# sushruta/uniformgrid-raytracing

Hardware: AMD Instinct MI355X
Metric: Mrays/s (primary+shadow+1-bounce) (higher is better)
Workload: dtype f32

## Files before the change

### uniformgrid-raytracing_amd/csrc/ugrt_context.hip

```cpp
#include "ugrt_ctx.h"

static int check_device(int device)
{
	int n = 0;
	hipError_t e = hipGetDeviceCount(&n);
	if (e != hipSuccess || n <= 0)
		return ugrt_fail(UGRT_ENODEV, "no HIP device available (%s); libugrt has no CPU fallback",
				 e != hipSuccess ? hipGetErrorString(e) : "device count 0");
	if (device < 0 || device >= n)
		return ugrt_fail(UGRT_EINVAL, "device %d out of range (%d devices)", device, n);
	return UGRT_OK;
}

int ugrt_buf_reserve(ugrt_ctx *ctx, DevBuf &b, size_t bytes)
{
	if (bytes <= b.cap && b.p)
		return UGRT_OK;
	size_t want = bytes + bytes / 2;
	if (want < 256)
		want = 256;
	void *np = nullptr;
	hipError_t e = hipMalloc(&np, want);
	if (e != hipSuccess)
		return ugrt_fail(UGRT_ENOMEM, "hipMalloc(%zu) failed: %s", want, hipGetErrorString(e));
// ... 145 lines not shown
	buf_free(ctx->pseg);
	buf_free(ctx->pbkt);
	buf_free(ctx->sray);
	if (ctx->h_pinned)
		(void)hipHostFree(ctx->h_pinned);
	if (ctx->d_small)
		(void)hipFree(ctx->d_small);
	for (int s = 0; s < UGRT_ST_COUNT; s++)
		for (auto &p : ctx->prof[s]) {
			(void)hipEventDestroy(p.a);
			(void)hipEventDestroy(p.b);
		}
	for (auto &p : ctx->prof_pool) {
		(void)hipEventDestroy(p.a);
		(void)hipEventDestroy(p.b);
	}
	delete ctx;
}

static const struct {
	const char *key;
	int lo, hi;
} k_opt[UGRT_OPT_COUNT] = {
	{ "dda_rays_per_wave", 0, 64 }, { "dda_coop", 1, 1 << 30 },     { "dda_kernel", 0, 1 },
	{ "dda_cull_min", 1, 1 << 30 }, { "dda_blocks", 1, 1 << 20 },
	{ "primary_seg", 64, 1 << 20 }, { "shadow_beam", 64, 8192 },
	{ "shadow_xseg", 64, 1 << 20 }, { "shadow_sizebits", 0, 8 },    { "shadow_itemsort", 0, 1 },
	{ "shadow_mbits", 1, 24 },      { "shadow_key64", 0, 1 },       { "sort_library", 0, 1 },
	{ "async_build", 0, 1 },        { "primary_waves", 64, 1 << 20 },
	{ "shadow_waves", 64, 1 << 20 }, { "dda_sort", 0, 1 }, { "primary_order", 0, 1 }, { "primary_chunk", 4, 64 }, { "sort_items", 8, 16 }, { "dda_cull_work", 1, 1 << 30 },
	{ "dda_split", 0, 4 }, { "dda_split_load", 50, 100000 }, { "dda_split_segments", 1, 4 }, { "primary_xcd_run", 0, 4096 }, { "shadow_xcd_run", 0, 4096 },
	{ "primary_centre", 0, 1 }, { "sort_rank", 0, 1 }, { "ray_sort", 0, 1 }, { "shadow_sieve", 0, 64 },
	{ "any_rays_per_wave", 0, 64 }, { "any_coop", 1, 1 << 30 }, { "uniform_reuse", 0, 1 },
	{ "light_reuse", 0, 1 }, { "shadow_pairs", 0, 1 },
};

extern "C" int ugrt_ctx_get_state(ugrt_ctx *ctx, const char *key, long long *value)
{
	if (!ctx || !key || !value)
		return ugrt_fail(UGRT_EINVAL, "ctx_get_state: null argument");
	if (strcmp(key, "radix_launches") == 0)
		*value = (long long)ctx->rs_launches;
	else if (strcmp(key, "sort_rank_atomic") == 0)
		*value = ctx->rs_atomic_rank < 0 ? -1 : (ctx->rs_atomic_rank == 1 && ctx->opt[UGRT_OPT_SORT_RANK] != 0 ? 1 : 0);
	else if (strcmp(key, "shadow_key_bits") == 0)
		*value = (long long)ctx->shadow_key_bits;
	else if (strcmp(key, "shadow_pairs_counted") == 0)
		*value = ctx->shadow_pairs_counted ? 1 : 0;
	else if (strcmp(key, "primary_deferred_merges") == 0)
		*value = (long long)ctx->merges_deferred;
	else if (strcmp(key, "primary_completed_merges") == 0)
		*value = (long long)ctx->merges_completed;
	else if (strcmp(key, "primary_merge_pending") == 0)
		*value = ctx->grid[UGRT_GRID_PERSPECTIVE].valid && ctx->grid[UGRT_GRID_PERSPECTIVE].merge_pending ? 1 : 0;
	else if (strcmp(key, "uniform_builds_reused") == 0)
		*value = (long long)ctx->uniform_reused;
	else if (strcmp(key, "light_builds_reused") == 0)
		*value = (long long)ctx->light_reused;
	else if (strcmp(key, "primary_slots_unarmed") == 0) {
		const size_t ncell = (size_t)ctx->nbx * (size_t)ctx->nby;
		std::vector<u64> b((size_t)ctx->npix);
		std::vector<u32> d(ncell);
		UGRT_HIP(hipSetDevice(ctx->device));
		UGRT_HIP(hipStreamSynchronize(ctx->stream));
		UGRT_HIP(hipMemcpy(b.data(), ctx->best.p, b.size() * sizeof(u64), hipMemcpyDeviceToHost));
		UGRT_HIP(hipMemcpy(d.data(), ctx->pdone.p, d.size() * sizeof(u32), hipMemcpyDeviceToHost));
		long long bad = 0;
		for (u64 v : b)
			bad += v != ~0ull;
		for (u32 v : d)
			bad += v != 0u;
		*value = bad;
	} else if (strcmp(key, "recip_mismatches") == 0) {
		unsigned long long bad = 0;
		const int rc = ugrt_recip_selftest(ctx, &bad);
		if (rc != UGRT_OK)
			return rc;
		*value = (long long)bad;
	} else if (strcmp(key, "f2i_mismatches") == 0) {
		unsigned long long bad = 0;
		const int rc = ugrt_f2i_selftest(ctx, &bad);
// ... 21 lines not shown
				return ugrt_fail(UGRT_EINVAL, "ctx_set_option: %s %d outside [%d,%d]", key, value, k_opt[i].lo,
						 k_opt[i].hi);
			ctx->opt[i] = (value < 0 || ((i == UGRT_OPT_DDA_RPW || i == UGRT_OPT_ANY_RPW) && value == 0)) ? -1 : value;
			return UGRT_OK;
		}
	return ugrt_fail(UGRT_EINVAL, "ctx_set_option: unknown key '%s'", key);
}

extern "C" int ugrt_ctx_set_stream(ugrt_ctx *ctx, void *hip_stream)
{
	if (!ctx)
		return ugrt_fail(UGRT_EINVAL, "set_stream: null ctx");
	UGRT_HIP(hipStreamSynchronize(ctx->stream));
	ctx->stream = (hipStream_t)hip_stream;
	return UGRT_OK;
}

extern "C" int ugrt_ctx_synchronize(ugrt_ctx *ctx)
{
	if (!ctx)
		return ugrt_fail(UGRT_EINVAL, "synchronize: null ctx");
	UGRT_HIP(hipStreamSynchronize(ctx->stream));
	if (ugrt_reported_status(ctx) != 0u || ctx->overflow_seen) {
		const unsigned bits = ugrt_reported_status(ctx);
		ctx->overflow_seen = false;
		for (int g = 0; g < 3; g++)
			ctx->h_pinned[UGRT_PIN_REPORT + 4 * g + 3] = 0u;
		ctx->h_pinned[UGRT_PIN_SHADOW + 2] = 0u;
		UGRT_HIP(hipMemsetAsync(ctx->d_small + UGRT_DSMALL_STATUS, 0, 4, ctx->stream));
		UGRT_HIP(hipStreamSynchronize(ctx->stream));
		for (int g = 0; g < 3; g++)
			ctx->grid[g].have_est = false;
		ctx->have_shadow_est = false;
		ctx->overflow_repair = true;
		return ugrt_fail(UGRT_EOVERFLOW, "an asynchronous call needed more room than its estimate gave it (status %u: "
						  "1 grid build, 2 shadow candidate pairs, 4 shadow work items): the frames since the last "
						  "synchronisation are incomplete, repeat them", bits);
	}
	ctx->overflow_repair = false;
	return UGRT_OK;
}

struct TexArg {
	float v[100];
};
__global__ void k_store_table(TexArg t, float *dst)
{
	int i = threadIdx.x;
	if (i < 100)
		dst[i] = t.v[i];
}

float *ugrt_ctx_tex(ugrt_ctx *ctx)
{
	float *dst = (float *)(ctx->d_small + UGRT_DSMALL_TEX);
	if (ctx->tex_dirty) {
		TexArg t;
		memcpy(t.v, ctx->tex_host, sizeof(t.v));
		hipLaunchKernelGGL(k_store_table, dim3(1), dim3(128), 0, ctx->stream, t, dst);
		ctx->tex_dirty = false;
	}
	return dst;
}

extern "C" int ugrt_upload_camera(ugrt_ctx *ctx, const float camcoords[64])
{
	if (!ctx || !camcoords)
		return ugrt_fail(UGRT_EINVAL, "upload_camera: null argument");
	memcpy(ctx->cam.cc, camcoords, sizeof(float) * 64);
// ... 149 lines not shown
```

### uniformgrid-raytracing_amd/csrc/ugrt_ctx.h

```cpp
#ifndef UGRT_CTX_H
#define UGRT_CTX_H

#include <hip/hip_runtime.h>

#include <vector>

#include "ugrt_internal.h"

struct CamBlock {
	float cc[64];
	float light[4];
	int W, H, nbx, nby;
	int strict_tex;
};

enum {
	UGRT_OPT_DDA_RPW = 0,
	UGRT_OPT_DDA_COOP,
	UGRT_OPT_DDA_KERNEL,
	UGRT_OPT_DDA_CULL_MIN,
	UGRT_OPT_DDA_BLOCKS,
	UGRT_OPT_PRIMARY_SEG,
	UGRT_OPT_SHADOW_BEAM,
	UGRT_OPT_SHADOW_XSEG,
	UGRT_OPT_SHADOW_SIZEBITS,
	UGRT_OPT_SHADOW_ITEMSORT,
	UGRT_OPT_SHADOW_MBITS,
	UGRT_OPT_SHADOW_KEY64,
	UGRT_OPT_SORT_LIBRARY,
	UGRT_OPT_ASYNC_BUILD,
	UGRT_OPT_PRIMARY_WAVES,
	UGRT_OPT_SHADOW_WAVES,
	UGRT_OPT_DDA_SORT,
	UGRT_OPT_PRIMARY_ORDER,
	UGRT_OPT_PRIMARY_CHUNK,
	UGRT_OPT_SORT_ITEMS,
	UGRT_OPT_DDA_CULL_WORK,
	UGRT_OPT_DDA_SPLIT,
	UGRT_OPT_DDA_SPLIT_LOAD,
	UGRT_OPT_DDA_SPLIT_SEGMENTS,
	UGRT_OPT_PRIMARY_XCD_RUN,
	UGRT_OPT_SHADOW_XCD_RUN,
	UGRT_OPT_PRIMARY_CENTRE,
	UGRT_OPT_SORT_RANK,
	UGRT_OPT_RAY_SORT,
	UGRT_OPT_SHADOW_SIEVE,
	UGRT_OPT_ANY_RPW,
	UGRT_OPT_ANY_COOP,
	UGRT_OPT_UNIFORM_REUSE,
	UGRT_OPT_LIGHT_REUSE,
	UGRT_OPT_SHADOW_PAIRS,
	UGRT_OPT_COUNT
};

struct DevBuf {
	void *p = nullptr;
	size_t cap = 0;
};

struct Grid;
struct BuildPlan {
	Grid *G;
	int F, ny, nz, ylo, yhi;
	u32 C;
	unsigned long long active;
	u32 Rn, W, R;
	u32 *rw;
	u32 *report, *status;
	bool no_wide;
	bool own_sort;
	bool prehist;
};

struct Grid {
	DevBuf rng, sizes, scan;
	DevBuf parts;
	DevBuf wide;
	DevBuf key[2], val[2];
	DevBuf span, offset;
	DevBuf projz;
	DevBuf uspan;
	int slabs = 1, F = 0;
	u32 est_rn = 0, est_w = 0;
	bool have_est = false, async_pending = false, r_exact = true;
	bool waited = false;
	unsigned long long active_cells = 0;
	u32 *keys = nullptr, *vals = nullptr;
	u32 R = 0, C = 0, cells_used = 0;
	int dims[3] = { 0, 0, 0 };
	float ug[12] = { 0 };
	bool valid = false;
	const u32 *wide_zeroed = nullptr;
	bool merge_pending = false;
	BuildPlan merge_plan = {};
};

#define UGRT_DSMALL_DDA_RAYS 2
#define UGRT_DSMALL_DDA_RAYS_B 4
#define UGRT_DSMALL_TICKET 8
#define UGRT_DSMALL_STATUS 14
#define UGRT_DSMALL_SHADOW_WORK 16
#define UGRT_DSMALL_PAIRS 20
#define UGRT_DSMALL_TEX 32
#define UGRT_DSMALL_DDA 132
#define UGRT_DSMALL_RW 236
#define UGRT_DSMALL_SHADOW 254
#define UGRT_DSMALL_PRIMARY 264
#define UGRT_DSMALL_WORDS (132 + 104 + 28 + 32)
#define UGRT_PIN_RW 0
#define UGRT_PIN_CELLS_USED 4
#define UGRT_PIN_REFS 8
#define UGRT_PIN_PAIRS 10
#define UGRT_PIN_CHUNKS 11
#define UGRT_PIN_BEAMS 12
#define UGRT_PIN_SHADOW_WORK (UGRT_PIN_SHADOW + 4)
#define UGRT_PIN_REPORT 32
#define UGRT_PIN_SHADOW 44
#define UGRT_PIN_WORDS 64
#define UGRT_STATUS_BUILD_OVERFLOW 1u
#define UGRT_STATUS_PAIR_OVERFLOW 2u
#define UGRT_STATUS_ITEM_OVERFLOW 4u
#define UGRT_DDA_STATS 46
#define UGRT_PRIMARY_STATS 16
static_assert(UGRT_DSMALL_DDA + 2 * UGRT_DDA_STATS <= UGRT_DSMALL_RW, "the DDA's counters run into the build counts");
static_assert(UGRT_DSMALL_RW + 6 <= UGRT_DSMALL_SHADOW && UGRT_DSMALL_SHADOW + 10 <= UGRT_DSMALL_PRIMARY && UGRT_DSMALL_PRIMARY + 2 * UGRT_PRIMARY_STATS <= UGRT_DSMALL_WORDS && UGRT_PIN_SHADOW + 8 <= UGRT_PIN_WORDS && UGRT_PIN_REPORT + 12 <= UGRT_PIN_SHADOW, "scratch layout");

struct ProfPair {
	hipEvent_t a, b;
};

struct ugrt_ctx {
	ugrt_config cfg;
	int device = 0;
	hipStream_t stream = nullptr;
	CamBlock cam;
	float tex_host[100];
	bool tex_dirty = false;
	int nbx = 0, nby = 0;
	int face_lo = 0, face_hi = -1;
	int p0 = 0, npix = 0;
	Grid grid[3];
	DevBuf temp;
	DevBuf scan_state;
	u32 scan_epoch = 0;
	DevBuf rs_state, rs_tmp[2][2];
	u32 rs_tiles = 0;
	u32 rs_epoch = 0;
	bool batch_open = false;
	int nbatch = 0;
	BuildPlan batch[2];
	unsigned long long rs_launches = 0;
	bool rs_prehist = false;
	int rs_atomic_rank = -1;
	DevBuf trirec;
	const float *rec_verts = nullptr;
	const int *rec_tris = nullptr;
	int rec_faces = 0;
	bool rec_valid = false;
// ... 13 lines not shown
	const u32 *ubitmap_span = nullptr;
	DevBuf witems, wscan;
	DevBuf ubitmap;
	DevBuf dsort;
	DevBuf dsplit;
	u32 dda_turn = 0;
	u32 dsplit_rpw = 0, dsplit_turn = 0;
	bool dda_deeper_level = false;
	DevBuf best;
	DevBuf pdone;
	DevBuf rmap[2];
	DevBuf rstart, cbase;
	DevBuf skey[2], sval[2], sdesc, sstart, sbase;
	DevBuf tkey[2], tval[2], tbcnt;
	DevBuf sray;
	DevBuf citem;
	DevBuf pseg;
	DevBuf pbkt;
	bool shadow_pairs_counted = false;
	DevBuf sitem;
	u32 *h_pinned = nullptr;
	u32 *d_small = nullptr;
	unsigned prof_mask = 0;
	unsigned chunk_capacity = 0;
	const unsigned *chunk_prefix = nullptr, *chunk_map = nullptr;
	bool ray_sort_pending = false;
	int opt[UGRT_OPT_COUNT];
	std::vector<ProfPair> prof[UGRT_ST_COUNT];
	std::vector<ProfPair> prof_pool;
	bool overflow_seen = false;
	bool overflow_repair = false;
	u32 est_pairs = 0, est_beams = 0;
	bool have_shadow_est = false, shadow_async_pending = false;
	u32 shadow_key_bits = 0;
	unsigned long long stats[8] = { 0 };
	unsigned long long dda_stats[UGRT_DDA_STATS] = { 0 };
	unsigned long long primary_stats[UGRT_PRIMARY_STATS] = { 0 };
	unsigned long long merges_deferred = 0, merges_completed = 0;
};

#define UGRT_HIP(call)                                                                            \
	do {                                                                                      \
		hipError_t e_ = (call);                                                           \
		if (e_ != hipSuccess)                                                             \
			return ugrt_fail(UGRT_EHIP, "%s:%d %s -> %s", __FILE__, __LINE__, #call, \
					 hipGetErrorString(e_));                                  \
	} while (0)

int ugrt_buf_reserve(ugrt_ctx *ctx, DevBuf &b, size_t bytes);
static inline const float4 *ugrt_trirec_of(const ugrt_ctx *ctx, const float *d_vertlist, const int *d_trilist)
{
	const bool use_rec = ctx->rec_valid && ctx->rec_verts == d_vertlist && ctx->rec_tris == d_trilist;
	return use_rec ? (const float4 *)ctx->trirec.p : (const float4 *)nullptr;
}
int ugrt_slab_union(ugrt_ctx *ctx, const u32 *d_span, const u32 *d_offset, u32 C, u32 slabs, const u32 **uspan,
		    const u32 **uoffset);
int ugrt_grid_complete(ugrt_ctx *ctx, Grid &G);
float *ugrt_ctx_tex(ugrt_ctx *ctx);
static inline u32 ugrt_reported_status(const ugrt_ctx *ctx)
{
	const u32 *p = ctx->h_pinned;
	return p[UGRT_PIN_REPORT + 3] | p[UGRT_PIN_REPORT + 7] | p[UGRT_PIN_REPORT + 11] | p[UGRT_PIN_SHADOW + 2];
}
void ugrt_prof_begin(ugrt_ctx *ctx, int stage);
void ugrt_prof_end(ugrt_ctx *ctx, int stage);

// ... 36 lines not shown
```

### uniformgrid-raytracing_amd/csrc/ugrt_trace_shadow.hip

```cpp
#include <algorithm>
#include <cstdlib>
#include "ugrt_packet.h"
#include "ugrt_rs_hist.h"
#include "ugrt_scan.h"
#ifndef GCHUNK
#define GCHUNK 32u
#endif

struct GBox {
	float cx, cy, cz;
	float rx, ry, rz;
	u32 ray_start;
	u32 ray_count;
};

__device__ __forceinline__ u32 d_spread10(u32 v)
{
	v &= 0x3FFu;
	v = (v | (v << 16)) & 0x030000FFu;
	v = (v | (v << 8)) & 0x0300F00Fu;
	v = (v | (v << 4)) & 0x030C30C3u;
	v = (v | (v << 2)) & 0x09249249u;
	return v;
}
// ... 81 lines not shown
		float tVal = t_value_list[pixel];
		float rd[3];
		rd[0] = (cmPt[0] + tVal * ray_direction_list[pixel * 3 + 0]) - cam.cc[0];
		rd[1] = (cmPt[1] + tVal * ray_direction_list[pixel * 3 + 1]) - cam.cc[1];
		rd[2] = (cmPt[2] + tVal * ray_direction_list[pixel * 3 + 2]) - cam.cc[2];
		D_NORMALIZE(rd);
		code = KEY64 ? d_dir_morton(rd) : d_dir_oct(rd, (mbits + 1u) / 2u, mbits / 2u);
	}
	if (KEY64)
		((u64 *)keys)[i] = ((u64)cell << 30) | (u64)code;
	else
		((u32 *)keys)[i] = key32 = (cell << mbits) | code;
	vals[i] = pixel;
	}
	if (!KEY64 && hs.hist)
		d_rs_count(s_rsh, key32 & 0xFFu, i < n);
	}
	__syncthreads();
	d_rs_flush(s_rsh, hs);
}

template <typename K>
__global__ __launch_bounds__(WL_THREADS) void k_shadow_runs(const K *__restrict__ keys, u32 n, u32 shift,
							     u32 *__restrict__ rstart, u32 *__restrict__ rend)
{
	u32 i = blockIdx.x * WL_THREADS + threadIdx.x;
	if (i >= n)
		return;
	u32 c = (u32)(keys[i] >> shift);
	if (i == 0 || (u32)(keys[i - 1] >> shift) != c)
		rstart[c] = i;
	if (i == n - 1 || (u32)(keys[i + 1] >> shift) != c)
		rend[c] = i + 1;
}

struct ShadowCountLoad {
	const u32 *span, *rstart, *rend;
	u32 beam;
	unsigned long long *tests;
	bool ITEMS;
	__device__ __forceinline__ void operator()(u32 base, u32 C, u32 (&v)[SC_ITEMS]) const
	{
#pragma unroll
		for (int k = 0; k < SC_ITEMS; k++) {
			const u32 c = base + (u32)k;
			u32 x = 0;
			if (c < C) {
				const u32 g = (rend[c] - rstart[c] + beam - 1u) / beam, sp = span[c];
				x = ITEMS ? (sp + 63u) / 64u * ((g + GCHUNK - 1) / GCHUNK) : g;
				if (!ITEMS && g && sp)
					atomicAdd(tests, (unsigned long long)sp * (unsigned long long)g);
			}
			v[k] = x;
		}
	}
};

__device__ __forceinline__ u32 d_find_cell(const u32 *__restrict__ incl, u32 C, u32 x)
{
	u32 lo = 0, hi = C - 1;
	while (lo < hi) {
		u32 mid = (lo + hi) >> 1;
		if (incl[mid] > x)
			hi = mid;
		else
			lo = mid + 1;
// ... 668 lines not shown
		if (ok) {
			const u32 pos = end - old + rank;
			if (pos < out_cap)
				pair_tri[pos] = tri;
		}
	}
}

#ifdef UGRT_SHADOW_TIMELINE
__device__ unsigned long long *g_shadow_tl;
#endif
template <bool REC>
__global__ __launch_bounds__(64) void k_trace_shadow(CamBlock cam, const u32 *__restrict__ xincl, u32 G,
						      const u32 *__restrict__ item_seg, const u32 *__restrict__ item_sub,
						      const GBox *__restrict__ boxes, const u32 *__restrict__ pstart,
						      const u32 *__restrict__ pend, const u32 *__restrict__ pair_tri,
						      const float *__restrict__ verts, const int *__restrict__ tris,
						      const float4 *__restrict__ rec, const float *__restrict__ t_value_list,
						      const float *__restrict__ ray_direction_list,
						      int *__restrict__ is_shadowed, const u32 *__restrict__ ray_pixels,
						      const float *__restrict__ cmPt, u32 XSEG, u32 *__restrict__ sub_done,
						      u32 nsubmax, const float4 *__restrict__ sray, u32 item_cap,
						      u32 *__restrict__ report, const u32 *__restrict__ status,
						      const unsigned long long *__restrict__ work, u32 SLICES, u32 W0, u32 SIEVE, u32 NSIEVE)
{
	__shared__ __attribute__((aligned(16))) float lds[64 * 16];
	const int lane = threadIdx.x;
#ifdef UGRT_SHADOW_TIMELINE
	const unsigned long long tl0 = __builtin_amdgcn_s_memrealtime();
	u32 tl_n = 0;
#endif
	if (blockIdx.x == 0 && lane == 0) {
		report[2] = *status;
		report[3] = 0u;
		reinterpret_cast<unsigned long long *>(report + 4)[0] = work[0];
		reinterpret_cast<unsigned long long *>(report + 4)[1] = work[1];
	}
	const u32 total = item_cap;
	const float lx = cam.cc[0], ly = cam.cc[1], lz = cam.cc[2];
	u32 first = blockIdx.x;
	if (SLICES == 1u) {
		first = d_xcd_block();
	} else if (SLICES > 1u) {
		const u32 rl = (SLICES >> 1) - 1u, j = blockIdx.x >> 3;
		first = ((((j >> rl) << 3) + (blockIdx.x & 7u)) << rl) + (j & ((1u << rl) - 1u));
	}
	const bool persistent = SLICES == 1u;
	for (u32 base = first; base < (persistent ? total : W0 + NSIEVE); base += gridDim.x) {
		const bool sieve = !persistent && base >= W0;
		const u32 n_v = sieve ? SIEVE : 1u, stride_v = sieve ? NSIEVE : 0u;
		u32 sgm_v = XSEG_LAST + 1u, gs_v = 0u;
		const u32 my_it = base + (u32)lane * stride_v;
		if ((u32)lane < n_v && my_it < total) {
			sgm_v = item_seg[my_it];
			gs_v = item_sub[my_it];
		}
		const u32 flagged_v = __hip_atomic_load(sub_done + (size_t)(gs_v >> 7) * nsubmax + (gs_v & 127u), __ATOMIC_RELAXED, __HIP_MEMORY_SCOPE_AGENT);
		unsigned long long todo = __ballot(sgm_v <= XSEG_LAST && flagged_v == 0u);
	while (todo != 0ull) {
#ifdef UGRT_SHADOW_TIMELINE
		tl_n++;
#endif
		const int tl = (int)__builtin_ctzll(todo);
		todo &= todo - 1ull;
		const u32 sgm = (u32)__builtin_amdgcn_readlane((int)sgm_v, tl), gs = (u32)__builtin_amdgcn_readlane((int)gs_v, tl);
		const u32 g = gs >> 7, sub = gs & 127u;
		u32 *my_done = sub_done + (size_t)g * nsubmax + sub;
// ... 101 lines not shown

static int bits_of(u32 v)
{
	int b = 1;
	while (b < 32 && (1ull << b) < (unsigned long long)v)
		b++;
	return b;
}

struct ShadowPass {
	ugrt_ctx *ctx;
	hipStream_t st;
	u32 C, n;
	const unsigned *d_value_list, *d_span, *d_offset, *d_map, *d_prefix_map;
	const float *d_vertlist, *d_t_value, *d_ray_dir, *d_cam_position;
	const int *d_trilist;
	int *d_is_shadowed;
	u32 ncellk;
	size_t maxg;
	u32 traced, launch_cap, nchunks_arg;
	const u32 *nchunks_dev;
	bool use_rec;
	const float4 *rec;
	void *k0, *k1;
	u32 *v0, *v1, *rstart, *rend, *gincl, *iincl, *pstart, *pend;
	GBox *boxes;
	unsigned long long *wcnt;
	bool own_sort, async;
	u32 beam, XSEG, sbits;
	u32 P, G, Gcap, xcap;
	const u32 *pgp;
	u32 *status, *report;
	u32 *xincl, *iseg1, *isub1;
	bool counted;
	u32 gbound, bkt_words, *bkt, *bincl, *segcnt, segcap;
	const u32 *pair_tri;
	int traced_chunks(unsigned num_chunks);
	int reserve();
	int plan();
	int beams();
	int cull();
	int candidates();
	int exact();
};

int ShadowPass::traced_chunks(unsigned num_chunks)
{
	const bool on_device = num_chunks == UGRT_CHUNKS_ON_DEVICE;
	launch_cap = (ctx->cfg.flags & UGRT_FLAG_SHADOW_ALL_CHUNKS) ? 0xFFFFFFFFu : (u32)ctx->nbx * (u32)ctx->nby;
	nchunks_arg = num_chunks;
	if (on_device) {
		if (!ctx->ray_sort_pending && !ctx->cbase.p)
			return ugrt_fail(UGRT_EINVAL, "trace_shadow: UGRT_CHUNKS_ON_DEVICE without a ugrt_sort_rays before");
		if (ctx->chunk_prefix != d_prefix_map || ctx->chunk_map != d_map)
			return ugrt_fail(UGRT_EINVAL, "trace_shadow: UGRT_CHUNKS_ON_DEVICE refers to the last ugrt_sort_rays, which "
						      "sorted other arrays");
		traced = num_chunks;
		if (ctx->ray_sort_pending)
			nchunks_arg = 0u;
		else
			nchunks_dev = (const u32 *)ctx->cbase.p + C;
	} else if (launch_cap == 0xFFFFFFFFu) {
		traced = num_chunks;
	} else {
		u32 lim = num_chunks < launch_cap ? num_chunks : launch_cap;
		traced = lim ? lim - 1 : 0;
	}
	ctx->stats[2] = traced;
	ctx->stats[1] = ctx->stats[6] = ctx->stats[7] = 0;
	return UGRT_OK;
}

int ShadowPass::reserve()
{
	int rc;
	if (ctx->cfg.slabs > 1 && (rc = ugrt_slab_union(ctx, d_span, d_offset, C, (u32)ctx->cfg.slabs, &d_span, &d_offset)))
		return rc;
	ncellk = C + 2;
	maxg = (size_t)n / 64 + C + 1;
	const struct { DevBuf &b; size_t bytes; } need[] = {
		{ ctx->skey[0], (size_t)n * 8 }, { ctx->sval[0], (size_t)n * 4 }, { ctx->skey[1], (size_t)n * 8 }, { ctx->sval[1], (size_t)n * 4 },
		{ ctx->sstart, (size_t)ncellk * 8 },
		{ ctx->sbase, (size_t)C * 8 },
		{ ctx->sdesc, maxg * sizeof(GBox) },
		{ ctx->tbcnt, maxg * 8 + maxg * 128 * 4 },
		{ ctx->witems, maxg * 8 },
		{ ctx->sray, (size_t)n * 16 },
		{ ctx->pseg, (size_t)PAIR_SEGS * PAIR_SEG_STRIDE * 4 },
	};
	for (const auto &r : need)
// ... 27 lines not shown
	if (async) {
		u32 gb = 1;
		while (gb < ctx->est_beams + ctx->est_beams / 4u + 1u)
			gb <<= 1;
		gbound = gb < gbound ? gb : gbound;
	}
	counted = ctx->opt[UGRT_OPT_SHADOW_PAIRS] != 0 && own_sort && ((unsigned long long)gbound << sbits) <= SHADOW_BUCKET_WORDS;
	ctx->shadow_pairs_counted = counted;
	if (counted) {
		bkt_words = gbound << sbits;
		const size_t half = ((size_t)bkt_words + 3u) / 4u * 4u;
		if ((rc = ugrt_buf_reserve(ctx, ctx->pbkt, 2 * half * 4)))
			return rc;
		bkt = (u32 *)ctx->pbkt.p, bincl = bkt + half;
	}
	return UGRT_OK;
}

int ShadowPass::beams()
{
	int rc;
	ugrt_prof_begin(ctx, UGRT_ST_SHADOW_PREP);
	const u32 cellbits = (u32)bits_of(ncellk);
	const bool key64 = cellbits > 20u || ctx->opt[UGRT_OPT_SHADOW_KEY64] == 1;
	u32 mbits = 32u - cellbits;
	if (ctx->opt[UGRT_OPT_SHADOW_MBITS] > 0 && (u32)ctx->opt[UGRT_OPT_SHADOW_MBITS] < mbits)
		mbits = (u32)ctx->opt[UGRT_OPT_SHADOW_MBITS];
	mbits = mbits > 24u ? 24u : mbits;
	ctx->shadow_key_bits = (key64 ? 30u : mbits) + cellbits;
	const u32 kblocks = (u32)((n + WL_THREADS - 1) / WL_THREADS) < 768u ? (u32)((n + WL_THREADS - 1) / WL_THREADS) : 768u;
	RsFirst hs = { nullptr };
	if (!key64 && own_sort && (rc = ugrt_sort_first_digit(ctx, &hs)))
		return rc;
	hipLaunchKernelGGL(key64 ? k_shadow_keys<true> : k_shadow_keys<false>, dim3(kblocks), dim3(WL_THREADS), 0, st,
			   ctx->cam, d_t_value, d_ray_dir, d_map, d_prefix_map, nchunks_arg, nchunks_arg ? traced : 0u, n, C, d_span,
			   d_cam_position, key64 ? 30u : mbits, k0, v0, rstart, 2u * ncellk, nchunks_dev, launch_cap, ctx->chunk_capacity,
			   (u32 *)wcnt, 5u, (u32 *)ctx->pseg.p, PAIR_SEGS * PAIR_SEG_STRIDE, hs);
	UGRT_HIP(hipGetLastError());
	if (key64)
		rc = ugrt_prim_sort_pairs64(ctx, (const u64 *)k0, (u64 *)k1, v0, v1, n, 30 + (int)cellbits);
	else
		rc = own_sort ? ugrt_sort_pairs_u32(ctx, (const u32 *)k0, (u32 *)k1, v0, v1, n, (int)(mbits + cellbits), nullptr, true)
			      : ugrt_prim_sort_pairs(ctx, (const u32 *)k0, (u32 *)k1, v0, v1, n, (int)(mbits + cellbits));
	if (rc)
		return rc;
	if (key64)
		hipLaunchKernelGGL(k_shadow_runs<u64>, dim3((n + WL_THREADS - 1) / WL_THREADS), dim3(WL_THREADS), 0, st,
				   (const u64 *)k1, n, 30u, rstart, rend);
	else
		hipLaunchKernelGGL(k_shadow_runs<u32>, dim3((n + WL_THREADS - 1) / WL_THREADS), dim3(WL_THREADS), 0, st,
				   (const u32 *)k1, n, mbits, rstart, rend);
	UGRT_HIP(hipGetLastError());
	beam = ctx->opt[UGRT_OPT_SHADOW_BEAM] > 0 ? (u32)ctx->opt[UGRT_OPT_SHADOW_BEAM] : 2048u;
	beam = beam < 64u ? 64u : (beam > 8192u ? 8192u : (beam + 63u) / 64u * 64u);
	XSEG = ctx->opt[UGRT_OPT_SHADOW_XSEG] > 0 ? (u32)ctx->opt[UGRT_OPT_SHADOW_XSEG] : 128u;
	XSEG = XSEG < 64u ? 64u : (XSEG + 63u) / 64u * 64u;
	const ShadowCountLoad nbeams = { d_span, rstart, rend, beam, wcnt, false }, nitems = { d_span, rstart, rend, beam, wcnt, true };
	if ((rc = ugrt_scan_launch_pair<true>(ctx, nbeams, gincl, nitems, iincl, C)))
		return rc;
	if ((rc = ugrt_buf_reserve(ctx, ctx->citem, (size_t)CULL_TABLE * sizeof(CullItem))))
		return rc;
	hipLaunchKernelGGL(k_shadow_boxes, dim3(launch_blocks_for((u32)maxg)), dim3(64 * BOX_WAVES), 0, st, ctx->cam,
			   (const u32 *)gincl, C, (const u32 *)rstart, (const u32 *)rend, (const u32 *)v1, d_t_value,
			   d_ray_dir, d_cam_position, boxes, beam, pstart, (u32)(2 * maxg + maxg * (beam / 64u)),
			   (float4 *)ctx->sray.p, (const u32 *)iincl, d_span, d_offset, (CullItem *)ctx->citem.p,
			   counted ? bkt : (u32 *)nullptr, bkt_words, sbits);
	UGRT_HIP(hipGetLastError());
	ugrt_prof_end(ctx, UGRT_ST_SHADOW_PREP);
	return UGRT_OK;
}

int ShadowPass::cull()
{
	int rc;
	u32 *pcount = ctx->d_small + UGRT_DSMALL_PAIRS;
	u32 *pg = ctx->d_small + UGRT_DSMALL_SHADOW;
	status = ctx->d_small + UGRT_DSMALL_STATUS, report = ctx->h_pinned + UGRT_PIN_SHADOW;
	xincl = (u32 *)ctx->witems.p;
	size_t cap, want = (size_t)4 << 22;
	if (async && ((size_t)ctx->est_pairs + ctx->est_pairs / 2 + 65536) * 4 > want)
		want = ((size_t)ctx->est_pairs + ctx->est_pairs / 2 + 65536) * 4;
	for (int attempt = 0; attempt < 3; attempt++) {
		if (ctx->tkey[0].cap / 4 * 4 < want &&
		    ((rc = ugrt_buf_reserve(ctx, ctx->tkey[0], want)) || (rc = ugrt_buf_reserve(ctx, ctx->tkey[1], want)) ||
		     (rc = ugrt_buf_reserve(ctx, ctx->tval[0], want)) || (rc = ugrt_buf_reserve(ctx, ctx->tval[1], want))))
// ... 33 lines not shown
		if (counted) {
			PairBucketLoad la = { bkt, segcnt, segcap, (const u32 *)(gincl + (C - 1)), async ? P : segcap * PAIR_SEGS, gbound, sbits, boxes,
					      wcnt + 1, XSEG, pcount, chk, false };
			PairBucketLoad lb = la;
			lb.ITEMS = true;
			ugrt_prof_begin(ctx, UGRT_ST_SHADOW_PREP);
			rc = ugrt_scan_launch_pair<true>(ctx, la, bincl, lb, xincl, bkt_words, async ? (size_t)gbound : maxg);
			ugrt_prof_end(ctx, UGRT_ST_SHADOW_PREP);
			if (rc)
				return rc;
		}
		if (async) {
			pgp = pg;
			xcap = (ctx->est_beams + ctx->est_beams / 4u + 64u + P / XSEG) * (beam / 64u);
			ctx->shadow_async_pending = true;
			break;
		}
		UGRT_HIP(hipMemcpyAsync(ctx->h_pinned + UGRT_PIN_PAIRS, pcount, 4, hipMemcpyDeviceToHost, st));
		UGRT_HIP(hipMemcpyAsync(ctx->h_pinned + UGRT_PIN_BEAMS, gincl + (C - 1), 4, hipMemcpyDeviceToHost, st));
		UGRT_HIP(hipStreamSynchronize(st));
		P = ctx->h_pinned[UGRT_PIN_PAIRS];
		if ((size_t)P <= cap)
			break;
		if (attempt == 2)
			return ugrt_fail(UGRT_ENOMEM, "trace_shadow: %u candidate pairs do not fit", P);
		want = (size_t)P * 4 + ((size_t)P * 4) / 4;
	}
	if (!async) {
		G = Gcap = ctx->h_pinned[UGRT_PIN_BEAMS];
		ctx->stats[1] = G;
		ctx->est_pairs = P;
		ctx->est_beams = G;
		ctx->have_shadow_est = true;
		ctx->h_pinned[UGRT_PIN_SHADOW] = P;
		ctx->h_pinned[UGRT_PIN_SHADOW + 1] = G;
		ctx->shadow_async_pending = false;
		xcap = (G + P / XSEG) * (beam / 64u);
	}
	return UGRT_OK;
}

int ShadowPass::candidates()
{
	int rc;
	ugrt_prof_begin(ctx, UGRT_ST_SHADOW_PREP);
	if (!counted) {
		if ((rc = own_sort ? ugrt_sort_pairs_u32(ctx, (const u32 *)ctx->tkey[0].p, (u32 *)ctx->tkey[1].p, (const u32 *)ctx->tval[0].p,
							 (u32 *)ctx->tval[1].p, P, bits_of(G) + (int)sbits, pgp, true)
				   : ugrt_prim_sort_pairs(ctx, (const u32 *)ctx->tkey[0].p, (u32 *)ctx->tkey[1].p, (const u32 *)ctx->tval[0].p,
							  (u32 *)ctx->tval[1].p, P, bits_of(G) + (int)sbits, pgp)))
			return rc;
		pair_tri = (const u32 *)ctx->tval[1].p;
		{
			u32 pb = (P + WL_THREADS - 1) / WL_THREADS;
			hipLaunchKernelGGL(k_pair_runs, dim3(pb ? pb : 1u), dim3(WL_THREADS), 0, st, (const u32 *)ctx->tkey[1].p, P, sbits,
					   pstart, pend, pgp);
		}
		UGRT_HIP(hipGetLastError());
		const PairItemLoad load = { pstart, pend, boxes, G, wcnt + 1, XSEG, pgp };
		if ((rc = ugrt_scan_launch<true>(ctx, load, xincl, Gcap, ScanTailNone())))
			return rc;
	}
	if ((rc = ugrt_buf_reserve(ctx, ctx->sitem, (size_t)xcap * 16)))
		return rc;
	u32 *iseg0 = (u32 *)ctx->sitem.p, *isub0 = iseg0 + xcap;
	iseg1 = isub0 + xcap, isub1 = iseg1 + xcap;
// ... 124 lines not shown
```

Measured before the change: 6226.

## Sort shadow rays as per-tile direction fragments instead of per-ray keys

```diff
diff --git a/uniformgrid-raytracing_amd/csrc/ugrt_context.hip b/uniformgrid-raytracing_amd/csrc/ugrt_context.hip
--- a/uniformgrid-raytracing_amd/csrc/ugrt_context.hip
+++ b/uniformgrid-raytracing_amd/csrc/ugrt_context.hip
@@ -201,7 +201,7 @@
 	{ "dda_split", 0, 4 }, { "dda_split_load", 50, 100000 }, { "dda_split_segments", 1, 4 }, { "primary_xcd_run", 0, 4096 }, { "shadow_xcd_run", 0, 4096 },
 	{ "primary_centre", 0, 1 }, { "sort_rank", 0, 1 }, { "ray_sort", 0, 1 }, { "shadow_sieve", 0, 64 },
 	{ "any_rays_per_wave", 0, 64 }, { "any_coop", 1, 1 << 30 }, { "uniform_reuse", 0, 1 },
-	{ "light_reuse", 0, 1 }, { "shadow_pairs", 0, 1 },
+	{ "light_reuse", 0, 1 }, { "shadow_pairs", 0, 1 }, { "shadow_frags", 0, 1 },
 };
 
 extern "C" int ugrt_ctx_get_state(ugrt_ctx *ctx, const char *key, long long *value)
@@ -216,6 +216,8 @@
 		*value = (long long)ctx->shadow_key_bits;
 	else if (strcmp(key, "shadow_pairs_counted") == 0)
 		*value = ctx->shadow_pairs_counted ? 1 : 0;
+	else if (strcmp(key, "shadow_fragments") == 0)
+		*value = ctx->shadow_frag_ran ? (long long)ctx->h_pinned[UGRT_PIN_SHADOW + 3] : 0;
 	else if (strcmp(key, "primary_deferred_merges") == 0)
 		*value = (long long)ctx->merges_deferred;
 	else if (strcmp(key, "primary_completed_merges") == 0)
@@ -303,9 +305,10 @@
 		for (int g = 0; g < 3; g++)
 			ctx->grid[g].have_est = false;
 		ctx->have_shadow_est = false;
+		ctx->have_frag_est = false;
 		ctx->overflow_repair = true;
 		return ugrt_fail(UGRT_EOVERFLOW, "an asynchronous call needed more room than its estimate gave it (status %u: "
-						  "1 grid build, 2 shadow candidate pairs, 4 shadow work items): the frames since the last "
+						  "1 grid build, 2 shadow candidate pairs, 4 shadow work items, 8 shadow fragments): the frames since the last "
 						  "synchronisation are incomplete, repeat them", bits);
 	}
 	ctx->overflow_repair = false;
diff --git a/uniformgrid-raytracing_amd/csrc/ugrt_ctx.h b/uniformgrid-raytracing_amd/csrc/ugrt_ctx.h
--- a/uniformgrid-raytracing_amd/csrc/ugrt_ctx.h
+++ b/uniformgrid-raytracing_amd/csrc/ugrt_ctx.h
@@ -50,6 +50,7 @@
 	UGRT_OPT_UNIFORM_REUSE,
 	UGRT_OPT_LIGHT_REUSE,
 	UGRT_OPT_SHADOW_PAIRS,
+	UGRT_OPT_SHADOW_FRAGS,
 	UGRT_OPT_COUNT
 };
 
@@ -106,7 +107,8 @@
 #define UGRT_DSMALL_RW 236
 #define UGRT_DSMALL_SHADOW 254
 #define UGRT_DSMALL_PRIMARY 264
-#define UGRT_DSMALL_WORDS (132 + 104 + 28 + 32)
+#define UGRT_DSMALL_FRAGS 296
+#define UGRT_DSMALL_WORDS (132 + 104 + 28 + 32 + 4)
 #define UGRT_PIN_RW 0
 #define UGRT_PIN_CELLS_USED 4
 #define UGRT_PIN_REFS 8
@@ -120,10 +122,11 @@
 #define UGRT_STATUS_BUILD_OVERFLOW 1u
 #define UGRT_STATUS_PAIR_OVERFLOW 2u
 #define UGRT_STATUS_ITEM_OVERFLOW 4u
+#define UGRT_STATUS_FRAG_OVERFLOW 8u
 #define UGRT_DDA_STATS 46
 #define UGRT_PRIMARY_STATS 16
 static_assert(UGRT_DSMALL_DDA + 2 * UGRT_DDA_STATS <= UGRT_DSMALL_RW, "the DDA's counters run into the build counts");
-static_assert(UGRT_DSMALL_RW + 6 <= UGRT_DSMALL_SHADOW && UGRT_DSMALL_SHADOW + 10 <= UGRT_DSMALL_PRIMARY && UGRT_DSMALL_PRIMARY + 2 * UGRT_PRIMARY_STATS <= UGRT_DSMALL_WORDS && UGRT_PIN_SHADOW + 8 <= UGRT_PIN_WORDS && UGRT_PIN_REPORT + 12 <= UGRT_PIN_SHADOW, "scratch layout");
+static_assert(UGRT_DSMALL_RW + 6 <= UGRT_DSMALL_SHADOW && UGRT_DSMALL_SHADOW + 10 <= UGRT_DSMALL_PRIMARY && UGRT_DSMALL_PRIMARY + 2 * UGRT_PRIMARY_STATS <= UGRT_DSMALL_FRAGS && UGRT_DSMALL_FRAGS + 3 <= UGRT_DSMALL_WORDS && UGRT_PIN_SHADOW + 8 <= UGRT_PIN_WORDS && UGRT_PIN_REPORT + 12 <= UGRT_PIN_SHADOW, "scratch layout");
 
 struct ProfPair {
 	hipEvent_t a, b;
@@ -203,6 +206,8 @@
 	bool overflow_repair = false;
 	u32 est_pairs = 0, est_beams = 0;
 	bool have_shadow_est = false, shadow_async_pending = false;
+	u32 est_frags = 0;
+	bool have_frag_est = false, shadow_frag_ran = false;
 	u32 shadow_key_bits = 0;
 	unsigned long long stats[8] = { 0 };
 	unsigned long long dda_stats[UGRT_DDA_STATS] = { 0 };
diff --git a/uniformgrid-raytracing_amd/csrc/ugrt_trace_shadow.hip b/uniformgrid-raytracing_amd/csrc/ugrt_trace_shadow.hip
--- a/uniformgrid-raytracing_amd/csrc/ugrt_trace_shadow.hip
+++ b/uniformgrid-raytracing_amd/csrc/ugrt_trace_shadow.hip
@@ -137,6 +137,209 @@
 		rstart[c] = i;
 	if (i == n - 1 || (u32)(keys[i + 1] >> shift) != c)
 		rend[c] = i + 1;
+}
+
+#define FRAG_BUF 1024u
+#ifndef FRAG_SPLIT_BITS
+#define FRAG_SPLIT_BITS 12u
+#endif
+#define FRAG_TILES 2u
+#define FRAG_ROUND (FRAG_TILES * (WL_THREADS / 64u))
+struct FragRec {
+	u32 tile, mask_lo, mask_hi, pad;
+};
+
+__global__ __launch_bounds__(WL_THREADS) void k_shadow_frags(CamBlock cam, const float *__restrict__ t_value_list,
+							      const float *__restrict__ ray_direction_list,
+							      const u32 *__restrict__ d_map, u32 n, u32 W, u32 C,
+							      const u32 *__restrict__ span, const float *__restrict__ cmPt, u32 mbits,
+							      u32 *__restrict__ keys, u32 *__restrict__ slots, FragRec *__restrict__ recs,
+							      u32 *__restrict__ fw, u32 cap, u32 *__restrict__ status, u32 *__restrict__ report,
+							      u32 *__restrict__ zero, u32 nzero, u32 *__restrict__ zero2, u32 nzero2,
+							      u32 *__restrict__ zero3, u32 nzero3, RsFirst hs)
+{
+	__shared__ u32 s_rsh[RS_BINS * RS_PRIV];
+	__shared__ u32 s_key[FRAG_BUF], s_tile[FRAG_BUF], s_mlo[FRAG_BUF], s_mhi[FRAG_BUF];
+	__shared__ u32 s_cnt, s_base;
+	for (u32 z = blockIdx.x * WL_THREADS + threadIdx.x; z < nzero; z += gridDim.x * WL_THREADS)
+		zero[z] = 0;
+	for (u32 z = blockIdx.x * WL_THREADS + threadIdx.x; z < nzero2; z += gridDim.x * WL_THREADS)
+		zero2[z] = 0;
+	for (u32 z = blockIdx.x * WL_THREADS + threadIdx.x; z < nzero3; z += gridDim.x * WL_THREADS)
+		zero3[z] = 0;
+	d_rs_zero(s_rsh, hs);
+	if (threadIdx.x == 0)
+		s_cnt = 0;
+	__syncthreads();
+	const u32 lane = threadIdx.x & 63u, wave = threadIdx.x >> 6;
+	const u32 ntiles = n >> 6, tilesx = W >> 3;
+	auto flush = [&]() {
+		const u32 cnt = s_cnt;
+		if (threadIdx.x == 0)
+			s_base = atomicAdd(&fw[0], cnt);
+		__syncthreads();
+		const u32 base = s_base;
+		for (u32 i0 = 0; i0 < cnt; i0 += WL_THREADS) {
+			const u32 i = i0 + threadIdx.x;
+			const bool ok = i < cnt && base + i < n;
+			u32 key = 0;
+			if (ok) {
+				key = s_key[i];
+				keys[base + i] = key;
+				slots[base + i] = base + i;
+				FragRec r = { s_tile[i], s_mlo[i], s_mhi[i], 0u };
+				recs[base + i] = r;
+			}
+			if (hs.hist)
+				d_rs_count(s_rsh, key & 0xFFu, ok);
+		}
+		__syncthreads();
+		if (threadIdx.x == 0)
+			s_cnt = 0;
+		__syncthreads();
+	};
+	for (u32 t0 = blockIdx.x * FRAG_ROUND; t0 < ntiles; t0 += gridDim.x * FRAG_ROUND) {
+		u32 tile[FRAG_TILES], pixel[FRAG_TILES], cell[FRAG_TILES];
+		bool live[FRAG_TILES];
+		float rd[FRAG_TILES][3];
+#pragma unroll
+		for (u32 u = 0; u < FRAG_TILES; u++) {
+			tile[u] = t0 + u * (WL_THREADS / 64u) + wave;
+			pixel[u] = 0u, cell[u] = C;
+			if (tile[u] < ntiles) {
+				const u32 ty = tile[u] / tilesx, tx = tile[u] - ty * tilesx;
+				const u32 i = (ty * 8u + (lane >> 3)) * W + tx * 8u + (lane & 7u);
+				pixel[u] = d_map[i];
+				cell[u] = d_map[n + i];
+			}
+		}
+#pragma unroll
+		for (u32 u = 0; u < FRAG_TILES; u++)
+			live[u] = cell[u] < C && span[cell[u] < C ? cell[u] : 0u] != 0u;
+#pragma unroll
+		for (u32 u = 0; u < FRAG_TILES; u++) {
+			rd[u][0] = rd[u][1] = rd[u][2] = 0.0f;
+			if (live[u]) {
+				const float tVal = t_value_list[pixel[u]];
+				rd[u][0] = (cmPt[0] + tVal * ray_direction_list[pixel[u] * 3 + 0]) - cam.cc[0];
+				rd[u][1] = (cmPt[1] + tVal * ray_direction_list[pixel[u] * 3 + 1]) - cam.cc[1];
+				rd[u][2] = (cmPt[2] + tVal * ray_direction_list[pixel[u] * 3 + 2]) - cam.cc[2];
+			}
+		}
+#pragma unroll
+		for (u32 u = 0; u < FRAG_TILES; u++) {
+			unsigned long long left = __ballot(live[u]), mine = 0ull;
+			if (left == 0ull)
+				continue;
+			D_NORMALIZE(rd[u]);
+			u32 nfrag = 0, rank = 0;
+			const u32 code = d_dir_oct(rd[u], (mbits + 1u) / 2u, mbits / 2u);
+			const u32 sb = FRAG_SPLIT_BITS < mbits ? FRAG_SPLIT_BITS : mbits;
+			const u32 part = (cell[u] << sb) | (code >> (mbits - sb));
+			while (left != 0ull) {
+				const u32 lead = (u32)__builtin_ctzll(left);
+				const u32 c = (u32)__builtin_amdgcn_readlane((int)part, (int)lead);
+				const unsigned long long same = __ballot(live[u] && part == c);
+				if (lane == lead) {
+					mine = same;
+					rank = nfrag;
+				}
+				nfrag++;
+				left &= ~same;
+			}
+			u32 base = 0;
+			if (lane == 0u)
+				base = atomicAdd(&s_cnt, nfrag);
+			base = (u32)__shfl((int)base, 0);
+			if (mine != 0ull) {
+				const u32 at = base + rank;
+				s_key[at] = (cell[u] << mbits) | code;
+				s_tile[at] = tile[u];
+				s_mlo[at] = (u32)mine;
+				s_mhi[at] = (u32)(mine >> 32);
+			}
+		}
+		__syncthreads();
+		if (s_cnt > FRAG_BUF - 64u * FRAG_ROUND)
+			flush();
+	}
+	if (s_cnt)
+		flush();
+	d_rs_flush(s_rsh, hs);
+	if (threadIdx.x == 0) {
+		asm volatile("s_waitcnt vmcnt(0)" ::: "memory");
+		if (atomicAdd(&fw[1], 1u) == gridDim.x - 1u) {
+			const u32 F = atomicExch(&fw[0], 0u);
+			fw[1] = 0u;
+			fw[2] = F <= cap ? F : 0u;
+			report[3] = F;
+			if (F > cap)
+				atomicOr(status, UGRT_STATUS_FRAG_OVERFLOW);
+		}
+	}
+}
+
+struct FragCountLoad {
+	const u32 *slots;
+	const FragRec *recs;
+	const u32 *count;
+	__device__ __forceinline__ void operator()(u32 base, u32 n, u32 (&v)[SC_ITEMS]) const
+	{
+		const u32 F = *count;
+		u32 s[SC_ITEMS];
+#pragma unroll
+		for (int k = 0; k < SC_ITEMS; k++)
+			s[k] = base + (u32)k < F && base + (u32)k < n ? slots[base + (u32)k] : 0xFFFFFFFFu;
+#pragma unroll
+		for (int k = 0; k < SC_ITEMS; k++) {
+			u32 x = 0;
+			if (s[k] != 0xFFFFFFFFu) {
+				const FragRec r = recs[s[k]];
+				x = (u32)__popc(r.mask_lo) + (u32)__popc(r.mask_hi);
+			}
+			v[k] = x;
+		}
+	}
+};
+
+#define FRAG_PER_WAVE 16u
+__global__ __launch_bounds__(WL_THREADS) void k_shadow_expand(const u32 *__restrict__ skeys, const u32 *__restrict__ slots,
+							       const FragRec *__restrict__ recs, const u32 *__restrict__ incl,
+							       const u32 *__restrict__ count, u32 mbits, const u32 *__restrict__ d_map, u32 n, u32 W,
+							       u32 *__restrict__ ray_pixels, u32 *__restrict__ rstart, u32 *__restrict__ rend)
+{
+	const u32 F = *count;
+	const u32 lane = threadIdx.x & 63u;
+	const u32 tilesx = W >> 3;
+	const u32 nwaves = gridDim.x * (WL_THREADS / 64u);
+	for (u32 j0 = (blockIdx.x * (WL_THREADS / 64u) + (threadIdx.x >> 6)) * FRAG_PER_WAVE; j0 < F; j0 += nwaves * FRAG_PER_WAVE) {
+		u32 tile = 0, mlo = 0, mhi = 0, first = 0;
+		const u32 j = j0 + lane;
+		if (lane < FRAG_PER_WAVE && j < F) {
+			const FragRec r = recs[slots[j]];
+			const u32 end = incl[j], c = skeys[j] >> mbits;
+			tile = r.tile, mlo = r.mask_lo, mhi = r.mask_hi;
+			first = end - ((u32)__popc(mlo) + (u32)__popc(mhi));
+			if (j == 0u || (skeys[j - 1u] >> mbits) != c)
+				rstart[c] = first;
+			if (j == F - 1u || (skeys[j + 1u] >> mbits) != c)
+				rend[c] = end;
+		}
+#pragma unroll
+		for (u32 k = 0; k < FRAG_PER_WAVE; k++) {
+			const u32 t = (u32)__builtin_amdgcn_readlane((int)tile, (int)k);
+			const u32 lo = (u32)__builtin_amdgcn_readlane((int)mlo, (int)k), hi = (u32)__builtin_amdgcn_readlane((int)mhi, (int)k);
+			const u32 at = (u32)__builtin_amdgcn_readlane((int)first, (int)k);
+			const unsigned long long mask = ((unsigned long long)hi << 32) | lo;
+			if ((mask >> lane) & 1ull) {
+				const u32 ty = t / tilesx, tx = t - ty * tilesx;
+				const u32 i = (ty * 8u + (lane >> 3)) * W + tx * 8u + (lane & 7u);
+				const u32 to = at + (u32)__popcll(mask & ((1ull << lane) - 1ull));
+				if (i < n && to < n)
+					ray_pixels[to] = d_map[i];
+			}
+		}
+	}
 }
 
 struct ShadowCountLoad {
@@ -871,7 +1074,6 @@
 #endif
 	if (blockIdx.x == 0 && lane == 0) {
 		report[2] = *status;
-		report[3] = 0u;
 		reinterpret_cast<unsigned long long *>(report + 4)[0] = work[0];
 		reinterpret_cast<unsigned long long *>(report + 4)[1] = work[1];
 	}
@@ -1039,6 +1241,7 @@
 	const u32 *pgp;
 	u32 *status, *report;
 	u32 *xincl, *iseg1, *isub1;
+	bool deferred;
 	bool counted;
 	u32 gbound, bkt_words, *bkt, *bincl, *segcnt, segcap;
 	const u32 *pair_tri;
@@ -1063,6 +1266,7 @@
 			return ugrt_fail(UGRT_EINVAL, "trace_shadow: UGRT_CHUNKS_ON_DEVICE refers to the last ugrt_sort_rays, which "
 						      "sorted other arrays");
 		traced = num_chunks;
+		deferred = ctx->ray_sort_pending;
 		if (ctx->ray_sort_pending)
 			nchunks_arg = 0u;
 		else
@@ -1156,6 +1360,41 @@
 	RsFirst hs = { nullptr };
 	if (!key64 && own_sort && (rc = ugrt_sort_first_digit(ctx, &hs)))
 		return rc;
+	const u32 W = (u32)ctx->cam.W;
+	const bool frags = deferred && !key64 && own_sort && ctx->opt[UGRT_OPT_SHADOW_FRAGS] != 0 && W != 0u && W % 8u == 0u &&
+			   n % (8u * W) == 0u;
+	ctx->shadow_frag_ran = frags;
+	if (frags) {
+		u32 *fw = ctx->d_small + UGRT_DSMALL_FRAGS;
+		u32 fcap = n;
+		if (async) {
+			if (ctx->have_frag_est) {
+				ctx->est_frags = ctx->h_pinned[UGRT_PIN_SHADOW + 3];
+				const unsigned long long want = (unsigned long long)ctx->est_frags + ctx->est_frags / 4u + 1024u;
+				fcap = want < n ? (u32)want : n;
+			} else {
+				ctx->h_pinned[UGRT_PIN_SHADOW + 3] = n;
+				ctx->have_frag_est = true;
+			}
+		}
+		u32 *fkeys = (u32 *)k0, *fincl = fkeys + n, *skeys = (u32 *)k1, *sslots = skeys + n;
+		FragRec *recs = (FragRec *)ctx->sray.p;
+		const u32 fb = (n / 64u + FRAG_ROUND - 1u) / FRAG_ROUND, fblocks = fb < 768u ? (fb ? fb : 1u) : 768u;
+		hipLaunchKernelGGL(k_shadow_frags, dim3(fblocks), dim3(WL_THREADS), 0, st, ctx->cam, d_t_value, d_ray_dir, d_map, n, W, C, d_span,
+				   d_cam_position, mbits, fkeys, v0, recs, fw, fcap, ctx->d_small + UGRT_DSMALL_STATUS,
+				   ctx->h_pinned + UGRT_PIN_SHADOW, rstart, 2u * ncellk, (u32 *)wcnt, 5u, (u32 *)ctx->pseg.p,
+				   PAIR_SEGS * PAIR_SEG_STRIDE, hs);
+		UGRT_HIP(hipGetLastError());
+		if ((rc = ugrt_sort_pairs_u32(ctx, fkeys, skeys, v0, sslots, fcap, (int)(mbits + cellbits), fw + 2, true)))
+			return rc;
+		const FragCountLoad nrays = { sslots, recs, fw + 2 };
+		if ((rc = ugrt_scan_launch<true>(ctx, nrays, fincl, fcap, ScanTailNone())))
+			return rc;
+		const u32 eb = (fcap + FRAG_PER_WAVE * (WL_THREADS / 64u) - 1u) / (FRAG_PER_WAVE * (WL_THREADS / 64u));
+		hipLaunchKernelGGL(k_shadow_expand, dim3(eb < 8192u ? (eb ? eb : 1u) : 8192u), dim3(WL_THREADS), 0, st, (const u32 *)skeys,
+				   (const u32 *)sslots, (const FragRec *)recs, (const u32 *)fincl, (const u32 *)(fw + 2), mbits, d_map, n, W, v1, rstart, rend);
+		UGRT_HIP(hipGetLastError());
+	} else {
 	hipLaunchKernelGGL(key64 ? k_shadow_keys<true> : k_shadow_keys<false>, dim3(kblocks), dim3(WL_THREADS), 0, st,
 			   ctx->cam, d_t_value, d_ray_dir, d_map, d_prefix_map, nchunks_arg, nchunks_arg ? traced : 0u, n, C, d_span,
 			   d_cam_position, key64 ? 30u : mbits, k0, v0, rstart, 2u * ncellk, nchunks_dev, launch_cap, ctx->chunk_capacity,
@@ -1175,6 +1414,7 @@
 		hipLaunchKernelGGL(k_shadow_runs<u32>, dim3((n + WL_THREADS - 1) / WL_THREADS), dim3(WL_THREADS), 0, st,
 				   (const u32 *)k1, n, mbits, rstart, rend);
 	UGRT_HIP(hipGetLastError());
+	}
 	beam = ctx->opt[UGRT_OPT_SHADOW_BEAM] > 0 ? (u32)ctx->opt[UGRT_OPT_SHADOW_BEAM] : 2048u;
 	beam = beam < 64u ? 64u : (beam > 8192u ? 8192u : (beam + 63u) / 64u * 64u);
 	XSEG = ctx->opt[UGRT_OPT_SHADOW_XSEG] > 0 ? (u32)ctx->opt[UGRT_OPT_SHADOW_XSEG] : 128u;
@@ -1274,6 +1514,8 @@
 		ctx->est_pairs = P;
 		ctx->est_beams = G;
 		ctx->have_shadow_est = true;
+		if (ctx->shadow_frag_ran)
+			ctx->have_frag_est = true;
 		ctx->h_pinned[UGRT_PIN_SHADOW] = P;
 		ctx->h_pinned[UGRT_PIN_SHADOW + 1] = G;
 		ctx->shadow_async_pending = false;
```

Result: faster. 6320, median of 6 (+1.5%).
